# RobotLocomotion/pytorch-dense-correspondence

Hardware: NVIDIA H100
Metric: image-pairs/s (640x480, D=3) fwd+loss+bwd (higher is better)
Workload: dtype f32 (bf16x3 split on the wgmma tensor cores, fp32 accumulate)

## Files before the change

pytorch-dense-correspondence_b200/csrc/conv_tc.cu:

```cuda
#include <cuda.h>
#include <algorithm>
#include <cstring>
#include <functional>
#include <mutex>
#include <unordered_map>

#include "conv.cuh"
#include "conv_tc.cuh"

namespace ddn {

constexpr int TC_BLOCK_K = 64;
constexpr int TC_CONSUMERS = 256;
constexpr int TC_THREADS = TC_CONSUMERS + 32;
constexpr int TC_PRODUCER_WARP = TC_CONSUMERS / 32;
constexpr int TC_WIDE_THREADS = TC_CONSUMERS + 128;
constexpr int TC_A_BYTES = 128 * TC_BLOCK_K * 2;

__device__ __forceinline__ uint32_t smem_u32(const void* p) { return (uint32_t)__cvta_generic_to_shared(p); }

__device__ __forceinline__ void mbar_init(uint32_t bar, uint32_t count) {
  asm volatile("mbarrier.init.shared::cta.b64 [%0], %1;" ::"r"(bar), "r"(count));
}
__device__ __forceinline__ void mbar_expect_tx(uint32_t bar, uint32_t bytes) {
// ... 2 lines not shown
__device__ __forceinline__ void mbar_arrive(uint32_t bar) {
  asm volatile("mbarrier.arrive.shared::cta.b64 _, [%0];" ::"r"(bar) : "memory");
}
__device__ __forceinline__ void mbar_wait(uint32_t bar, uint32_t parity) {
  asm volatile(
      "{\n\t"
      ".reg .pred p;\n\t"
      "WAIT_LOOP:\n\t"
      "mbarrier.try_wait.parity.shared::cta.b64 p, [%0], %1;\n\t"
      "@p bra WAIT_DONE;\n\t"
      "bra WAIT_LOOP;\n\t"
      "WAIT_DONE:\n\t"
      "}\n" ::"r"(bar), "r"(parity) : "memory");
}
__device__ __forceinline__ void fence_barrier_init() { asm volatile("fence.mbarrier_init.release.cluster;" ::: "memory"); }

__device__ __forceinline__ void tma_load_4d(uint32_t dst, const CUtensorMap* map, uint32_t bar, int c0, int c1, int c2, int c3) {
  asm volatile(
      "cp.async.bulk.tensor.4d.shared::cluster.global.mbarrier::complete_tx::bytes [%0], [%1, {%3, %4, %5, %6}], [%2];"
      ::"r"(dst), "l"(map), "r"(bar), "r"(c0), "r"(c1), "r"(c2), "r"(c3) : "memory");
}
__device__ __forceinline__ void tma_load_2d(uint32_t dst, const CUtensorMap* map, uint32_t bar, int c0, int c1) {
  asm volatile(
      "cp.async.bulk.tensor.2d.shared::cluster.global.mbarrier::complete_tx::bytes [%0], [%1, {%3, %4}], [%2];"
      ::"r"(dst), "l"(map), "r"(bar), "r"(c0), "r"(c1) : "memory");
}
__device__ __forceinline__ void tma_prefetch_l2_4d(const CUtensorMap* map, int c0, int c1, int c2, int c3) {
  asm volatile("cp.async.bulk.prefetch.tensor.4d.L2.global.tile [%0, {%1, %2, %3, %4}];" ::"l"(map), "r"(c0), "r"(c1), "r"(c2), "r"(c3) : "memory");
}
__device__ __forceinline__ void tma_prefetch_desc(const CUtensorMap* map) {
  asm volatile("prefetch.tensormap [%0];" ::"l"(map) : "memory");
}

__device__ __forceinline__ uint64_t gmma_desc(uint32_t smem_addr, uint32_t lbo_bytes, uint32_t sbo_bytes) {
  return (uint64_t)((smem_addr >> 4) & 0x3FFF) | ((uint64_t)((lbo_bytes >> 4) & 0x3FFF) << 16) |
         ((uint64_t)((sbo_bytes >> 4) & 0x3FFF) << 32) | ((uint64_t)1 << 62);
}
__device__ __forceinline__ uint64_t gmma_desc_k(uint32_t smem_addr, uint32_t sbo_bytes = 1024) { return gmma_desc(smem_addr, 16, sbo_bytes); }

template <int R>
__device__ __forceinline__ void setmaxnreg_dec() { asm volatile("setmaxnreg.dec.sync.aligned.u32 %0;" ::"n"(R)); }
template <int R>
__device__ __forceinline__ void setmaxnreg_inc() { asm volatile("setmaxnreg.inc.sync.aligned.u32 %0;" ::"n"(R)); }
__device__ __forceinline__ void wgmma_fence() { asm volatile("wgmma.fence.sync.aligned;" ::: "memory"); }
__device__ __forceinline__ void wgmma_commit() { asm volatile("wgmma.commit_group.sync.aligned;" ::: "memory"); }
template <int N>
__device__ __forceinline__ void wgmma_wait() { asm volatile("wgmma.wait_group.sync.aligned %0;" ::"n"(N) : "memory"); }
template <int K>
__device__ __forceinline__ void fence_acc(float (&d)[K]) {
#pragma unroll
  for (int i = 0; i < K; ++i) asm volatile("" : "+f"(d[i])::"memory");
}

template <int N> struct Wgmma;
template <> struct Wgmma<32> {
  template <int TRANS>
  static __device__ __forceinline__ void mma(float (&d)[16], uint64_t a, uint64_t b, int scale_d) {
    asm volatile(
        "{\n.reg .pred p;\nsetp.ne.b32 p, %18, 0;\n"
        "wgmma.mma_async.sync.aligned.m64n32k16.f32.bf16.bf16 {"
        "%0, %1, %2, %3, %4, %5, %6, %7, %8, %9, %10, %11, %12, %13, %14, %15"
        "}, %16, %17, p, 1, 1, %19, %19;\n}\n"
        : "+f"(d[0]), "+f"(d[1]), "+f"(d[2]), "+f"(d[3]), "+f"(d[4]), "+f"(d[5]), "+f"(d[6]), "+f"(d[7]),
          "+f"(d[8]), "+f"(d[9]), "+f"(d[10]), "+f"(d[11]), "+f"(d[12]), "+f"(d[13]), "+f"(d[14]), "+f"(d[15])
        : "l"(a), "l"(b), "r"(scale_d), "n"(TRANS));
  }
};
template <> struct Wgmma<64> {
  template <int TRANS>
// ... 160 lines not shown
        if (!(fmaf(rw[i].x - mu.x, scl.x, be.x) > 0.f)) g.x = 0.f;
        if (!(fmaf(rw[i].y - mu.y, scl.y, be.y) > 0.f)) g.y = 0.f;
        if (!(fmaf(rw[i].z - mu.z, scl.z, be.z) > 0.f)) g.z = 0.f;
        if (!(fmaf(rw[i].w - mu.w, scl.w, be.w) > 0.f)) g.w = 0.f;
      }
      s1.x += g.x; s1.y += g.y; s1.z += g.z; s1.w += g.w;
      s2.x = fmaf(g.x, (rw[i].x - mu.x) * is.x, s2.x); s2.y = fmaf(g.y, (rw[i].y - mu.y) * is.y, s2.y);
      s2.z = fmaf(g.z, (rw[i].z - mu.z) * is.z, s2.z); s2.w = fmaf(g.w, (rw[i].w - mu.w) * is.w, s2.w);
    }
  } else {
#pragma unroll
    for (int i = 0; i < EPI_ROWS; ++i) {
      const float4 raw = i < n_ok ? v[i] : make_float4(0.f, 0.f, 0.f, 0.f);
      if (i < n_ok)
        *reinterpret_cast<float4*>(p.out + off + i * rs) = make_float4(raw.x + adv[i].x, raw.y + adv[i].y, raw.z + adv[i].z, raw.w + adv[i].w);
      s1.x += raw.x; s1.y += raw.y; s1.z += raw.z; s1.w += raw.w;
      s2.x = fmaf(raw.x, raw.x, s2.x); s2.y = fmaf(raw.y, raw.y, s2.y); s2.z = fmaf(raw.z, raw.z, s2.z); s2.w = fmaf(raw.w, raw.w, s2.w);
    }
  }
}

__device__ __forceinline__ void colsum_lane_groups(float4& s1, float4& s2) {
#pragma unroll
  for (int off = 8; off < 32; off <<= 1) {
    s1.x += __shfl_xor_sync(0xffffffffu, s1.x, off); s1.y += __shfl_xor_sync(0xffffffffu, s1.y, off);
    s1.z += __shfl_xor_sync(0xffffffffu, s1.z, off); s1.w += __shfl_xor_sync(0xffffffffu, s1.w, off);
    s2.x += __shfl_xor_sync(0xffffffffu, s2.x, off); s2.y += __shfl_xor_sync(0xffffffffu, s2.y, off);
    s2.z += __shfl_xor_sync(0xffffffffu, s2.z, off); s2.w += __shfl_xor_sync(0xffffffffu, s2.w, off);
  }
}

__device__ __forceinline__ void named_barrier(int id, int threads) { asm volatile("bar.sync %0, %1;" ::"r"(id), "r"(threads) : "memory"); }

__device__ __forceinline__ void conv_epilogue_finalize(const TcEpilogueParams& p, int C, int* s_last, int bar) {
  if (p.fin.a.acc) {
    if (bn_last_cta(p.fin.a.ticket, gridDim.x, threadIdx.x == 0, s_last, [bar] { named_barrier(bar, TC_CONSUMERS); }))
      for (int c = threadIdx.x; c < C; c += TC_CONSUMERS) bn_fwd_finalize_channel(p.fin, c);
  } else if (p.bst.fin.a.acc) {
    if (bn_last_cta(p.bst.fin.a.ticket, gridDim.x, threadIdx.x == 0, s_last, [bar] { named_barrier(bar, TC_CONSUMERS); }))
      for (int c = threadIdx.x; c < C; c += TC_CONSUMERS) bn_bwd_finalize_channel(p.bst.fin, c);
  }
}

struct TcConvParams {
  TcEpilogueParams epi;
  int N, H, W, Cin, Cout;
  int taps_w;
  int dil;
  int stride;
  int tiles_h, tiles_w;
  int n_sub;
  int n_co;
  int full_items, tail_split, total_items;
};

constexpr int TC_SUB_H = 4, TC_SUB_W = 16;
constexpr int TC_SUB_BYTES = 64 * 128;

struct TcItem { int sp, co0, width; };
__device__ __forceinline__ TcItem tc_item(const TcConvParams& p, int idx, int block_n) {
  int tile = idx, piece = 0, width = block_n;
  if (idx >= p.full_items) {
    const int j = idx - p.full_items;
    tile = p.full_items + j / p.tail_split;
    piece = j - (j / p.tail_split) * p.tail_split;
    width = block_n / p.tail_split;
  }
  TcItem it;
  it.sp = tile / p.n_co;
  it.co0 = (tile - it.sp * p.n_co) * block_n + piece * width;
  it.width = width;
  return it;
}
struct TcSub { int n, h0, w0; bool valid; };
__device__ __forceinline__ TcSub tc_sub(const TcConvParams& p, int st) {
  TcSub s;
  s.valid = st < p.n_sub;
  const int tw = st % p.tiles_w; const int t = st / p.tiles_w;
  const int th = t % p.tiles_h;
  s.n = s.valid ? t / p.tiles_h : p.N;
  s.h0 = th * TC_SUB_H; s.w0 = tw * TC_SUB_W;
  return s;
}

template <int W, int BLOCK_N, int NPROD, int STAGES, int TRANS = 0>
__device__ __forceinline__ void conv_tc_mainloop(float (&acc)[W / 2], float (&accx)[W / 2], int num_kb, uint32_t& g, const uint64_t* full_bar,
                                                 const uint64_t* empty_bar, const uint8_t* smem, int wg, int lane) {
  constexpr int NSPLIT = NPROD == 3 ? 2 : 1;
  constexpr int A_BYTES = 128 * TC_BLOCK_K * 2;
  constexpr int B_BYTES = BLOCK_N * TC_BLOCK_K * 2;
  constexpr int STAGE_BYTES = NSPLIT * (A_BYTES + B_BYTES);
  constexpr uint32_t LBO = TRANS ? TC_SUB_BYTES : 16;
  constexpr int K_STEP = TRANS ? 16 * 128 : 32;
  for (int kb = 0; kb < num_kb; ++kb, ++g) {
    const int s = g % STAGES;
    mbar_wait(smem_u32(&full_bar[s]), (g / STAGES) & 1);
    wgmma_fence();
    const uint32_t stg = smem_u32(smem + (size_t)s * STAGE_BYTES);
    const uint64_t a_hi = gmma_desc(stg + wg * TC_SUB_BYTES, LBO, 1024), a_lo = gmma_desc(stg + A_BYTES + wg * TC_SUB_BYTES, LBO, 1024);
    const uint64_t b_hi = gmma_desc(stg + NSPLIT * A_BYTES, LBO, 1024), b_lo = gmma_desc(stg + 2 * A_BYTES + B_BYTES, LBO, 1024);
#pragma unroll
    for (int k = 0; k < TC_BLOCK_K / 16; ++k) {
      const uint64_t adv = (uint64_t)((k * K_STEP) >> 4);
      mma_k16_x<W, TRANS, NPROD>(acc, accx, a_hi + adv, a_lo + adv, b_hi + adv, b_lo + adv, (kb | k) != 0);
    }
    wgmma_commit();
    wgmma_wait<1>();
    if (kb > 0 && lane == 0) mbar_arrive(smem_u32(&empty_bar[(g - 1) % STAGES]));
  }
  wgmma_wait<0>();
  fence_acc(acc);
  if (NPROD == 3) { fence_acc(accx); add_cross(acc, accx); }
  if (lane == 0) mbar_arrive(smem_u32(&empty_bar[(g - 1) % STAGES]));
}

template <int BLOCK_N, int NPROD>
__global__ void __launch_bounds__(TC_WIDE_THREADS, 1)
conv_tc_kernel(const __grid_constant__ CUtensorMap tm_a_hi, const __grid_constant__ CUtensorMap tm_a_lo,
               const __grid_constant__ CUtensorMap tm_b_hi, const __grid_constant__ CUtensorMap tm_b_lo,
               const __grid_constant__ CUtensorMap tm_bt_hi, const __grid_constant__ CUtensorMap tm_bt_lo,
               const TcConvParams p) {
  constexpr int NSPLIT = NPROD == 3 ? 2 : 1;
  constexpr int A_BYTES = 128 * TC_BLOCK_K * 2;
  constexpr int B_BYTES = BLOCK_N * TC_BLOCK_K * 2;
  constexpr int STAGE_BYTES = NSPLIT * (A_BYTES + B_BYTES);
  constexpr int STAGES = (192 * 1024) / STAGE_BYTES >= 8 ? 8 : (192 * 1024) / STAGE_BYTES;
  static_assert(STAGES >= 2, "pipeline needs at least two stages");

  extern __shared__ __align__(1024) uint8_t smem_raw[];
  uint8_t* smem = reinterpret_cast<uint8_t*>((reinterpret_cast<uintptr_t>(smem_raw) + 1023) & ~uintptr_t(1023));
  __shared__ __align__(8) uint64_t full_bar[STAGES];
  __shared__ __align__(8) uint64_t empty_bar[STAGES];
  __shared__ int s_last;
  __shared__ __align__(16) float s_stage[TC_CONSUMERS / 32][EPI_WARP_FLOATS];
  __shared__ __align__(16) float s_part[2][2][4][BLOCK_N];
// ... 68 lines not shown
      const int n_ok = (sb.valid && h < p.H) ? min(EPI_ROWS, p.W - w4) : 0;
      const size_t pix = ((size_t)(n_ok > 0 ? sb.n : 0) * p.H + (n_ok > 0 ? h : 0)) * p.W + (n_ok > 0 ? w4 : 0);
      const size_t cbase = pix * p.Cout + it.co0 + gb * 4;
      const int grp = sb.valid ? sb.n / p.epi.imgs_per_group : 0;
#pragma unroll
      for (int c = 0; c < BLOCK_N / 32; ++c) {
        if (c < (it.width >> 5)) {
          float4 v[EPI_ROWS];
          stage_chunk(acc, c, st, lane, v);
          float4 s1 = make_float4(0.f, 0.f, 0.f, 0.f), s2 = s1;
          conv_epilogue_rows(p.epi, v, cbase + c * 32, (size_t)p.Cout, n_ok, it.co0 + c * 32 + gb * 4, p.Cout, grp, s1, s2);
          if (stats || bstats) {
            colsum_lane_groups(s1, s2);
            if (ga == 0) {
              *reinterpret_cast<float4*>(&s_part[wg][0][w][c * 32 + gb * 4]) = s1;
              *reinterpret_cast<float4*>(&s_part[wg][1][w][c * 32 + gb * 4]) = s2;
            }
          }
        }
      }
      if (stats || bstats) {
        named_barrier(1 + wg, 128);
        if (sb.valid)
          for (int col = e; col < it.width; col += 128) {
#pragma unroll
            for (int k = 0; k < 2; ++k) {
              const float sum = s_part[wg][k][0][col] + s_part[wg][k][1][col] + s_part[wg][k][2][col] + s_part[wg][k][3][col];
              red_add_f64(sum_acc + (size_t)(grp * 2 + k) * p.Cout + it.co0 + col, (double)sum);
            }
          }
        named_barrier(1 + wg, 128);
      }
    }
    conv_epilogue_finalize(p.epi, p.Cout, &s_last, 3);
  }
}

struct TcHaloParams {
  TcEpilogueParams epi;
  int N, H, W;
  int tiles_h, tiles_w, n_tiles;
};
constexpr int HALO_TH = 8, HALO_TW = 16;
constexpr int HALO_BH = HALO_TH + 2, HALO_BW = HALO_TW + 2;
constexpr int HALO_BOX_BYTES = HALO_BH * HALO_BW * 128;
constexpr int HALO_SLOT = ((HALO_BOX_BYTES + 1023) / 1024) * 1024;
constexpr int HALO_B_TAP = 64 * 128;
constexpr int HALO_B_PLANE = 9 * HALO_B_TAP;
__host__ __device__ constexpr int halo_slots(int nprod) { return nprod == 3 ? 2 : 3; }

template <int NPROD>
__global__ void __launch_bounds__(TC_THREADS, 1)
conv64_halo_kernel(const __grid_constant__ CUtensorMap tm_a_hi, const __grid_constant__ CUtensorMap tm_a_lo,
                   const __grid_constant__ CUtensorMap tm_b_hi, const __grid_constant__ CUtensorMap tm_b_lo, const TcHaloParams p) {
  constexpr int NSPLIT = NPROD == 3 ? 2 : 1;
  constexpr int SLOTS = halo_slots(NPROD);
  extern __shared__ __align__(1024) uint8_t smem_raw[];
  uint8_t* smem = reinterpret_cast<uint8_t*>((reinterpret_cast<uintptr_t>(smem_raw) + 1023) & ~uintptr_t(1023));
  uint8_t* smem_b = smem;
  uint8_t* smem_a = smem + NSPLIT * HALO_B_PLANE;
  __shared__ __align__(8) uint64_t full_bar[SLOTS], empty_bar[SLOTS], b_full;
  __shared__ int s_last;
  __shared__ __align__(16) float s_stage[TC_CONSUMERS / 32][EPI_WARP_FLOATS];
  __shared__ __align__(16) float s_part[2][8][64];

  pdl_trigger();
  const int warp = __shfl_sync(0xffffffffu, threadIdx.x >> 5, 0), lane = threadIdx.x & 31;
// ... 108 lines not shown
      fence_acc(acc);
      if (NPROD == 3) { fence_acc(accx); add_cross(acc, accx); }
      if (lane == 0) mbar_arrive(smem_u32(&empty_bar[(g - 1) % SLOTS]));

      const size_t pix0 = ((size_t)n * p.H + h0 + EPI_ROWS * (ga & 1)) * p.W + (w0 + 8 * wg + 2 * w + (ga >> 1));
      const size_t row_stride = (size_t)p.W * 64;
      const int grp = n / p.epi.imgs_per_group;
#pragma unroll
      for (int c = 0; c < 2; ++c) {
        float4 v[EPI_ROWS];
        stage_chunk(acc, c, st, lane, v);
        float4 s1 = make_float4(0.f, 0.f, 0.f, 0.f), s2 = s1;
        conv_epilogue_rows(p.epi, v, pix0 * 64 + gb * 4 + c * 32, row_stride, EPI_ROWS, c * 32 + gb * 4, 64, grp, s1, s2);
        if (stats || bstats) {
          colsum_lane_groups(s1, s2);
          if (ga == 0) {
            *reinterpret_cast<float4*>(&s_part[0][warp][c * 32 + gb * 4]) = s1;
            *reinterpret_cast<float4*>(&s_part[1][warp][c * 32 + gb * 4]) = s2;
          }
        }
      }
      if (stats || bstats) {
        named_barrier(3, TC_CONSUMERS);
        if (threadIdx.x < 128) {
          const int col = threadIdx.x & 63, k = threadIdx.x >> 6;
          float s8 = 0.f;
#pragma unroll
          for (int q = 0; q < 8; ++q) s8 += s_part[k][q][col];
          red_add_f64(sum_acc + (size_t)(grp * 2 + k) * 64 + col, (double)s8);
        }
        named_barrier(3, TC_CONSUMERS);
      }
    }
    conv_epilogue_finalize(p.epi, 64, &s_last, 3);
  }
}

struct TcWgradParams {
  double* dwp;
  int N, H, W, Cin, Cout;
  int taps_w, dil, stride;
  int tiles_h, tiles_w;
  int total_kb;
  int n_co, n_ci, n_tiles;
  int chunks;
};

struct WgradItem { int co0, ci0, tap, kb0, kb1; };
__device__ __forceinline__ WgradItem wgrad_item(const TcWgradParams& p, int idx, int bn) {
  const int c = idx / p.n_tiles;
  int t = idx - c * p.n_tiles;
  WgradItem it;
  it.co0 = (t % p.n_co) * 128; t /= p.n_co;
  it.ci0 = (t % p.n_ci) * bn;
  it.tap = t / p.n_ci;
  it.kb0 = (int)((int64_t)c * p.total_kb / p.chunks);
  it.kb1 = (int)((int64_t)(c + 1) * p.total_kb / p.chunks);
  return it;
}

template <int BN, int NPROD>
__global__ void __launch_bounds__(TC_WIDE_THREADS, 1)
wgrad_tc_kernel(const __grid_constant__ CUtensorMap tm_dy_hi, const __grid_constant__ CUtensorMap tm_dy_lo,
                const __grid_constant__ CUtensorMap tm_x_hi, const __grid_constant__ CUtensorMap tm_x_lo,
                const TcWgradParams p) {
  constexpr int NSPLIT = NPROD == 3 ? 2 : 1;
  constexpr int B_BYTES = BN * TC_BLOCK_K * 2;
// ... 407 lines not shown
                                  const cuuint32_t*, const cuuint32_t*, CUtensorMapInterleave, CUtensorMapSwizzle,
                                  CUtensorMapL2promotion, CUtensorMapFloatOOBfill);

static EncodeTiledFn get_encode_fn() {
  static EncodeTiledFn fn = nullptr;
  static bool tried = false;
  if (!tried) {
    tried = true;
    void* p = nullptr;
    cudaDriverEntryPointQueryResult qres;
    if (cudaGetDriverEntryPoint("cuTensorMapEncodeTiled", &p, cudaEnableDefault, &qres) == cudaSuccess &&
        qres == cudaDriverEntryPointSuccess)
      fn = (EncodeTiledFn)p;
  }
  return fn;
}

struct MapKey {
  const void* base; int d0, d1, d2, d3, b0, b1, b2, sample;
  bool operator==(const MapKey& o) const {
    return base == o.base && d0 == o.d0 && d1 == o.d1 && d2 == o.d2 && d3 == o.d3 && b0 == o.b0 && b1 == o.b1 && b2 == o.b2 && sample == o.sample;
  }
};
struct MapKeyHash {
  size_t operator()(const MapKey& k) const {
    size_t h = std::hash<const void*>()(k.base);
    for (int v : {k.d0, k.d1, k.d2, k.d3, k.b0, k.b1, k.b2, k.sample}) h = h * 1000003u ^ (size_t)v;
    return h;
  }
};
static std::unordered_map<MapKey, CUtensorMap, MapKeyHash> g_maps;
static std::mutex g_maps_mu;

static int make_act_map(CUtensorMap* m, const void* base, int N, int H, int W, int C, int sample = 1) {
  const MapKey key = {base, C, W, H, N, TC_BLOCK_K, TC_SUB_W, TC_SUB_H, sample};
  {
    std::lock_guard<std::mutex> lk(g_maps_mu);
    auto it = g_maps.find(key);
    if (it != g_maps.end()) { *m = it->second; return 0; }
  }
  EncodeTiledFn enc = get_encode_fn();
  if (!enc) { set_error("cuTensorMapEncodeTiled is unavailable (driver too old?)"); return DDN_EUNSUPPORTED; }
  cuuint64_t dims[4] = {(cuuint64_t)C, (cuuint64_t)W, (cuuint64_t)H, (cuuint64_t)N};
  cuuint64_t strides[3] = {(cuuint64_t)C * 2, (cuuint64_t)W * C * 2, (cuuint64_t)H * W * C * 2};
  cuuint32_t box[4] = {(cuuint32_t)TC_BLOCK_K, (cuuint32_t)(TC_SUB_W * sample), (cuuint32_t)(TC_SUB_H * sample), 1};
  cuuint32_t es[4] = {1, (cuuint32_t)sample, (cuuint32_t)sample, 1};
  CUresult r = enc(m, CU_TENSOR_MAP_DATA_TYPE_BFLOAT16, 4, const_cast<void*>(base), dims, strides, box, es,
                   CU_TENSOR_MAP_INTERLEAVE_NONE, CU_TENSOR_MAP_SWIZZLE_128B, CU_TENSOR_MAP_L2_PROMOTION_L2_128B,
                   CU_TENSOR_MAP_FLOAT_OOB_FILL_NONE);
  if (r != CUDA_SUCCESS) { set_error("cuTensorMapEncodeTiled(activations) failed: %d", (int)r); return DDN_EINVAL; }
  std::lock_guard<std::mutex> lk(g_maps_mu);
  if (g_maps.size() > 8192) g_maps.clear();
  g_maps[key] = *m;
  return 0;
}
static int make_act_map_hw(CUtensorMap* m, const void* base, int N, int H, int W, int C, int box_h, int box_w) {
  const MapKey key = {base, C, H, W, N, TC_BLOCK_K, box_h, box_w, -2};
  {
    std::lock_guard<std::mutex> lk(g_maps_mu);
    auto it = g_maps.find(key);
    if (it != g_maps.end()) { *m = it->second; return 0; }
  }
  EncodeTiledFn enc = get_encode_fn();
  if (!enc) { set_error("cuTensorMapEncodeTiled is unavailable (driver too old?)"); return DDN_EUNSUPPORTED; }
  cuuint64_t dims[4] = {(cuuint64_t)C, (cuuint64_t)H, (cuuint64_t)W, (cuuint64_t)N};
  cuuint64_t strides[3] = {(cuuint64_t)W * C * 2, (cuuint64_t)C * 2, (cuuint64_t)H * W * C * 2};
  cuuint32_t box[4] = {(cuuint32_t)TC_BLOCK_K, (cuuint32_t)box_h, (cuuint32_t)box_w, 1};
  cuuint32_t es[4] = {1, 1, 1, 1};
  CUresult r = enc(m, CU_TENSOR_MAP_DATA_TYPE_BFLOAT16, 4, const_cast<void*>(base), dims, strides, box, es,
                   CU_TENSOR_MAP_INTERLEAVE_NONE, CU_TENSOR_MAP_SWIZZLE_128B, CU_TENSOR_MAP_L2_PROMOTION_L2_128B,
                   CU_TENSOR_MAP_FLOAT_OOB_FILL_NONE);
  if (r != CUDA_SUCCESS) { set_error("cuTensorMapEncodeTiled(halo activations) failed: %d", (int)r); return DDN_EINVAL; }
  std::lock_guard<std::mutex> lk(g_maps_mu);
  if (g_maps.size() > 8192) g_maps.clear();
  g_maps[key] = *m;
  return 0;
}
static int make_act_map_halo(CUtensorMap* m, const void* base, int N, int H, int W, int C) {
  return make_act_map_hw(m, base, N, H, W, C, HALO_BH, HALO_BW);
}
static int make_weight_map(CUtensorMap* m, const void* base, int rows, int K, int box_rows) {
  const MapKey key = {base, K, rows, 0, 0, TC_BLOCK_K, box_rows, 0, -1};
  {
    std::lock_guard<std::mutex> lk(g_maps_mu);
    auto it = g_maps.find(key);
    if (it != g_maps.end()) { *m = it->second; return 0; }
  }
  EncodeTiledFn enc = get_encode_fn();
  if (!enc) { set_error("cuTensorMapEncodeTiled is unavailable (driver too old?)"); return DDN_EUNSUPPORTED; }
  cuuint64_t dims[2] = {(cuuint64_t)K, (cuuint64_t)rows};
  cuuint64_t strides[1] = {(cuuint64_t)K * 2};
  cuuint32_t box[2] = {(cuuint32_t)TC_BLOCK_K, (cuuint32_t)box_rows};
  cuuint32_t es[2] = {1, 1};
  CUresult r = enc(m, CU_TENSOR_MAP_DATA_TYPE_BFLOAT16, 2, const_cast<void*>(base), dims, strides, box, es,
                   CU_TENSOR_MAP_INTERLEAVE_NONE, CU_TENSOR_MAP_SWIZZLE_128B, CU_TENSOR_MAP_L2_PROMOTION_L2_256B,
                   CU_TENSOR_MAP_FLOAT_OOB_FILL_NONE);
  if (r != CUDA_SUCCESS) { set_error("cuTensorMapEncodeTiled(weights) failed: %d", (int)r); return DDN_EINVAL; }
  std::lock_guard<std::mutex> lk(g_maps_mu);
  if (g_maps.size() > 8192) g_maps.clear();
  g_maps[key] = *m;
  return 0;
}

template <int BN, int NPROD>
static int launch_wgrad_tc(const CUtensorMap& dy_hi, const CUtensorMap& dy_lo, const CUtensorMap& x_hi, const CUtensorMap& x_lo,
                           const TcWgradParams& p, int workers, cudaStream_t st) {
  constexpr int NSPLIT = NPROD == 3 ? 2 : 1;
  constexpr int STAGE_BYTES = NSPLIT * (TC_A_BYTES + BN * TC_BLOCK_K * 2);
  constexpr int STAGES = (192 * 1024) / STAGE_BYTES >= 8 ? 8 : (192 * 1024) / STAGE_BYTES;
  const size_t smem = (size_t)STAGES * STAGE_BYTES + 1024;
  static bool configured = false;
  if (!configured) {
    DDN_CUDA(cudaFuncSetAttribute(wgrad_tc_kernel<BN, NPROD>, cudaFuncAttributeMaxDynamicSharedMemorySize, (int)smem));
    configured = true;
  }
  DDN_LAUNCH((wgrad_tc_kernel<BN, NPROD>), workers, TC_WIDE_THREADS, smem, st, dy_hi, dy_lo, x_hi, x_lo, p);
  return 0;
}

static int tc_wgrad_chunks(int tiles, int total_kb, int workers) {
  const double even = (double)tiles * total_kb / workers;
  const int max_s = std::max(1, total_kb / 4);
  int best = 1;
  double best_span = 1e300;
  for (int s = 1; s <= max_s; ++s) {
    const double span = (double)ceil_div((int64_t)s * tiles, workers) * (double)ceil_div(total_kb, s);
    if (span <= 1.02 * even) return s;
    if (span < best_span) { best_span = span; best = s; }
// ... 99 lines not shown

int tc_upsample_zero_split(const float* dy, __nv_bfloat16* hi, __nv_bfloat16* lo, int N, int Ho, int Wo, int C, int precision,
                           cudaStream_t st) {
  int64_t total = (int64_t)N * Ho * Wo * (C / 4);
  int blocks = (int)std::min<int64_t>(ceil_div(total, 256), (int64_t)num_sms() * 8);
  DDN_LAUNCH(upsample_zero_split_kernel, blocks, 256, 0, st, dy, hi, lo, N, Ho, Wo, C, precision == DDN_PRECISION_BF16X3 ? 1 : 0);
  return 0;
}

int tc_stem_patches(const float* x_nchw, __nv_bfloat16* hi, __nv_bfloat16* lo, int N, int H, int W, int precision, cudaStream_t st) {
  const int H1 = (H - 1) / 2 + 1, W1 = (W - 1) / 2 + 1;
  DDN_CHECK_ARG(N <= 65535 && H1 <= 65535, "stem: batch / height too large for the launch grid");
  dim3 grid((unsigned)ceil_div(W1, STEM_TW), (unsigned)H1, (unsigned)N);
  DDN_LAUNCH(stem_patch_split_kernel, grid, 256, 0, st, x_nchw, hi, lo, N, H, W, H1, W1, precision == DDN_PRECISION_BF16X3 ? 1 : 0);
  return 0;
}

template <int BLOCK_N, int NPROD>
static int launch_conv_tc(const CUtensorMap& a_hi, const CUtensorMap& a_lo, const CUtensorMap& b_hi, const CUtensorMap& b_lo,
                          const CUtensorMap& bt_hi, const CUtensorMap& bt_lo, const TcConvParams& p, int workers, cudaStream_t st) {
  constexpr int NSPLIT = NPROD == 3 ? 2 : 1;
  constexpr int STAGE_BYTES = NSPLIT * (128 * TC_BLOCK_K * 2 + BLOCK_N * TC_BLOCK_K * 2);
  constexpr int STAGES = (192 * 1024) / STAGE_BYTES >= 8 ? 8 : (192 * 1024) / STAGE_BYTES;
  const size_t smem = (size_t)STAGES * STAGE_BYTES + 1024;
  static bool configured = false;
  if (!configured) {
    DDN_CUDA(cudaFuncSetAttribute(conv_tc_kernel<BLOCK_N, NPROD>, cudaFuncAttributeMaxDynamicSharedMemorySize, (int)smem));
    configured = true;
  }
  DDN_LAUNCH((conv_tc_kernel<BLOCK_N, NPROD>), workers, TC_WIDE_THREADS, smem, st, a_hi, a_lo, b_hi, b_lo, bt_hi, bt_lo, p);
  return 0;
}

template <int NPROD>
static int launch_conv64_halo(const CUtensorMap& a_hi, const CUtensorMap& a_lo, const CUtensorMap& b_hi, const CUtensorMap& b_lo,
                              const TcHaloParams& p, cudaStream_t st) {
  constexpr int NSPLIT = NPROD == 3 ? 2 : 1;
  const size_t smem = (size_t)NSPLIT * HALO_B_PLANE + (size_t)halo_slots(NPROD) * HALO_SLOT + 1024;
  static bool configured = false;
  if (!configured) {
    DDN_CUDA(cudaFuncSetAttribute(conv64_halo_kernel<NPROD>, cudaFuncAttributeMaxDynamicSharedMemorySize, (int)smem));
    configured = true;
  }
  const int grid = std::min(p.n_tiles, tc_worker_sms());
  DDN_LAUNCH((conv64_halo_kernel<NPROD>), grid, TC_THREADS, smem, st, a_hi, a_lo, b_hi, b_lo, p);
  return 0;
}

static int tc_epilogue_request(TcEpilogueParams* e, float* out, const float* addend, const BnFwdFinal* stats, const TcBwdStats* bst,
                               const TcFoldedEpilogue* ep, int N, int gout, int dgrad, int want_lo) {
  memset(e, 0, sizeof(*e));
  e->out = out; e->addend = addend; e->imgs_per_group = N;
  if (stats) {
    DDN_CHECK_ARG(!dgrad && !ep && stats->G >= 1 && stats->G <= BN_MAX_GROUPS && N % stats->G == 0 && stats->C == gout,
                  "bad BatchNorm statistics request");
    e->fin = *stats;
    e->imgs_per_group = N / stats->G;
  }
  if (bst) {
    DDN_CHECK_ARG(dgrad && !ep && !stats && bst->raw && bst->mean && bst->invstd && bst->fin.a.acc && bst->fin.G >= 1 &&
                  bst->fin.G <= BN_MAX_GROUPS && N % bst->fin.G == 0 && bst->fin.C == gout && (bst->y_hi || !bst->relu || (bst->gamma && bst->beta)),
                  "bad BatchNorm backward-statistics request");
    e->bst = *bst;
    e->imgs_per_group = N / bst->fin.G;
  }
  if (ep) {
// ... 32 lines not shown
  if (k == 3 && gin == 64 && gout == 64 && stride == 1 && dil == 1 && Ho % HALO_TH == 0 && Wo % HALO_TW == 0) {
    TcHaloParams hp;
    memset(&hp, 0, sizeof(hp));
    hp.epi = epi; hp.N = N; hp.H = Ho; hp.W = Wo;
    hp.tiles_h = Ho / HALO_TH; hp.tiles_w = Wo / HALO_TW; hp.n_tiles = N * hp.tiles_h * hp.tiles_w;
    CUtensorMap ma_hi, ma_lo, mb_hi, mb_lo;
    DDN_TRY(make_act_map_halo(&ma_hi, in.hi, N, H, W, 64));
    DDN_TRY(make_act_map_halo(&ma_lo, want_lo ? in.lo : in.hi, N, H, W, 64));
    DDN_TRY(make_weight_map(&mb_hi, b_hi, 64, 9 * 64, 64));
    DDN_TRY(make_weight_map(&mb_lo, want_lo ? b_lo : b_hi, 64, 9 * 64, 64));
    ProfScope ps(dgrad ? PROF_CONV_DGRAD_TC : PROF_CONV_FWD_TC, fl, st);
    return want_lo ? launch_conv64_halo<3>(ma_hi, ma_lo, mb_hi, mb_lo, hp, st) : launch_conv64_halo<1>(ma_hi, ma_lo, mb_hi, mb_lo, hp, st);
  }
  const int block_n = gout % 128 == 0 ? 128 : 64;
  TcConvParams p;
  memset(&p, 0, sizeof(p));
  p.epi = epi; p.N = N; p.H = Ho; p.W = Wo; p.Cin = gin; p.Cout = gout; p.taps_w = k; p.dil = dil;
  p.stride = stride;
  p.tiles_h = (int)ceil_div(Ho, TC_SUB_H); p.tiles_w = (int)ceil_div(Wo, TC_SUB_W);
  p.n_sub = N * p.tiles_h * p.tiles_w;
  p.n_co = gout / block_n;
  const int tiles = (int)ceil_div(p.n_sub, 2) * p.n_co;
  const int workers_max = tc_worker_sms();
  const int rem = tiles % workers_max;
  int split = 1;
  if (rem)
    while (split * 2 <= 8 && block_n / (split * 2) >= 32 && rem * split * 2 <= workers_max) split *= 2;
  p.full_items = tiles - rem; p.tail_split = split; p.total_items = p.full_items + rem * split;
  if (split == 1) { p.full_items = tiles; p.total_items = tiles; }
  const int workers = std::min(p.total_items, workers_max);
  const int b_rows = block_n;
  const int bt_rows = b_rows / split;
  CUtensorMap ma_hi, ma_lo, mb_hi, mb_lo, mt_hi, mt_lo;
  DDN_TRY(make_act_map(&ma_hi, in.hi, N, H, W, gin, stride));
  DDN_TRY(make_act_map(&ma_lo, want_lo ? in.lo : in.hi, N, H, W, gin, stride));
  DDN_TRY(make_weight_map(&mb_hi, b_hi, gout, k * k * gin, b_rows));
  DDN_TRY(make_weight_map(&mb_lo, want_lo ? b_lo : b_hi, gout, k * k * gin, b_rows));
  DDN_TRY(make_weight_map(&mt_hi, b_hi, gout, k * k * gin, bt_rows));
  DDN_TRY(make_weight_map(&mt_lo, want_lo ? b_lo : b_hi, gout, k * k * gin, bt_rows));
  ProfScope ps(dgrad ? PROF_CONV_DGRAD_TC : PROF_CONV_FWD_TC, fl, st);
#define CONV_TC(BN)                                                                                                           \
  (want_lo ? launch_conv_tc<BN, 3>(ma_hi, ma_lo, mb_hi, mb_lo, mt_hi, mt_lo, p, workers, st)                                   \
           : launch_conv_tc<BN, 1>(ma_hi, ma_lo, mb_hi, mb_lo, mt_hi, mt_lo, p, workers, st))
  if (block_n == 128) return CONV_TC(128);
  return CONV_TC(64);
#undef CONV_TC
}

int tc_dgrad_strided(const float* dy_f32, TcPlanes up, const float* w_oihw, const TcPlanes* w_packed, float* dx, const float* addend,
                     int N, int H, int W, int Cin, int Cout, int k, int precision, void* wws, size_t wws_bytes, cudaStream_t st,
                     const TcBwdStats* bst) {
  DDN_TRY(tc_upsample_zero_split(dy_f32, const_cast<__nv_bfloat16*>(up.hi), const_cast<__nv_bfloat16*>(up.lo), N, H / 2, W / 2, Cout,
                                 precision, st));
  return tc_conv_planes(up, w_oihw, w_packed, dx, addend, nullptr, N, H, W, Cin, Cout, k, 1, 1, 1, precision, wws, wws_bytes, st, nullptr, bst);
}

int tc_stem_pack_weights(const float* w_conv1, __nv_bfloat16* hi, __nv_bfloat16* lo, int precision, cudaStream_t st) {
  DDN_LAUNCH(stem_pack_weights_kernel, (64 * 192 + 255) / 256, 256, 0, st, w_conv1, hi, lo, precision == DDN_PRECISION_BF16X3 ? 1 : 0);
  return 0;
}
int tc_stem_forward(TcPlanes patches, const float* w_conv1, const TcPlanes* w_packed, float* raw, const BnFwdFinal* stats, int N, int H1,
                    int W1, int precision, void* wws, size_t wws_bytes, cudaStream_t st) {
  TcPlanes wpk;
  if (w_packed) wpk = *w_packed;
  else {
    char* base = reinterpret_cast<char*>(align_up(reinterpret_cast<uintptr_t>(wws), 1024));
    DDN_CHECK_ARG((size_t)(base - (char*)wws) + 2 * 64 * 192 * 2 + 1024 <= wws_bytes, "weight staging too small");
    __nv_bfloat16* ph = (__nv_bfloat16*)base; __nv_bfloat16* pl = (__nv_bfloat16*)(base + align_up((size_t)64 * 192 * 2, 1024));
    DDN_TRY(tc_stem_pack_weights(w_conv1, ph, pl, precision, st));
    wpk.hi = ph; wpk.lo = pl;
  }
  return tc_conv_planes(patches, nullptr, &wpk, raw, nullptr, stats, N, H1, W1, 192, 64, 1, 1, 1, 0, precision, wws, wws_bytes, st);
}

int tc_stem_wgrad(TcPlanes patches, TcPlanes dy, int N, int H1, int W1, int precision, double* dwp, cudaStream_t st) {
  return tc_wgrad_planes(patches, dy, nullptr, N, H1, W1, 192, 64, 1, 1, 1, precision, dwp, st);
}

// ... 61 lines not shown
```

Before: 140.6.

## Add dgrad conv kernel with dedicated epilogue warpgroup via smem handoff

Adds a warp-specialized dgrad convolution kernel in which two consumer warpgroups run the wgmma mainloop and a separate epilogue warpgroup drains accumulators from a shared-memory handoff buffer. This lets the epilogue (stores, BN stats reduction) overlap the next tile's MMA work. To fit the handoff buffer and a deep ring, the k-block shrinks to 32 channels with 64B swizzle TMA maps and matching wgmma descriptors. The costs are a lower MMA-per-barrier ratio, extra shared-memory traffic for the handoff, and tighter register budgets.

```diff
diff --git a/pytorch-dense-correspondence_b200/csrc/conv_tc.cu b/pytorch-dense-correspondence_b200/csrc/conv_tc.cu
--- a/pytorch-dense-correspondence_b200/csrc/conv_tc.cu
+++ b/pytorch-dense-correspondence_b200/csrc/conv_tc.cu
@@ -58,9 +58,9 @@
   asm volatile("prefetch.tensormap [%0];" ::"l"(map) : "memory");
 }
 
-__device__ __forceinline__ uint64_t gmma_desc(uint32_t smem_addr, uint32_t lbo_bytes, uint32_t sbo_bytes) {
+__device__ __forceinline__ uint64_t gmma_desc(uint32_t smem_addr, uint32_t lbo_bytes, uint32_t sbo_bytes, uint32_t layout = 1) {
   return (uint64_t)((smem_addr >> 4) & 0x3FFF) | ((uint64_t)((lbo_bytes >> 4) & 0x3FFF) << 16) |
-         ((uint64_t)((sbo_bytes >> 4) & 0x3FFF) << 32) | ((uint64_t)1 << 62);
+         ((uint64_t)((sbo_bytes >> 4) & 0x3FFF) << 32) | ((uint64_t)layout << 62);
 }
 __device__ __forceinline__ uint64_t gmma_desc_k(uint32_t smem_addr, uint32_t sbo_bytes = 1024) { return gmma_desc(smem_addr, 16, sbo_bytes); }
 
@@ -287,13 +287,13 @@
 
 __device__ __forceinline__ void named_barrier(int id, int threads) { asm volatile("bar.sync %0, %1;" ::"r"(id), "r"(threads) : "memory"); }
 
-__device__ __forceinline__ void conv_epilogue_finalize(const TcEpilogueParams& p, int C, int* s_last, int bar) {
+__device__ __forceinline__ void conv_epilogue_finalize(const TcEpilogueParams& p, int C, int* s_last, int bar, int tid, int nthreads) {
   if (p.fin.a.acc) {
-    if (bn_last_cta(p.fin.a.ticket, gridDim.x, threadIdx.x == 0, s_last, [bar] { named_barrier(bar, TC_CONSUMERS); }))
-      for (int c = threadIdx.x; c < C; c += TC_CONSUMERS) bn_fwd_finalize_channel(p.fin, c);
+    if (bn_last_cta(p.fin.a.ticket, gridDim.x, tid == 0, s_last, [bar, nthreads] { named_barrier(bar, nthreads); }))
+      for (int c = tid; c < C; c += nthreads) bn_fwd_finalize_channel(p.fin, c);
   } else if (p.bst.fin.a.acc) {
-    if (bn_last_cta(p.bst.fin.a.ticket, gridDim.x, threadIdx.x == 0, s_last, [bar] { named_barrier(bar, TC_CONSUMERS); }))
-      for (int c = threadIdx.x; c < C; c += TC_CONSUMERS) bn_bwd_finalize_channel(p.bst.fin, c);
+    if (bn_last_cta(p.bst.fin.a.ticket, gridDim.x, tid == 0, s_last, [bar, nthreads] { named_barrier(bar, nthreads); }))
+      for (int c = tid; c < C; c += nthreads) bn_bwd_finalize_channel(p.bst.fin, c);
   }
 }
 
@@ -338,24 +338,27 @@
   return s;
 }
 
-template <int W, int BLOCK_N, int NPROD, int STAGES, int TRANS = 0>
+template <int W, int BLOCK_N, int NPROD, int STAGES, int TRANS = 0, int BLOCK_K = TC_BLOCK_K>
 __device__ __forceinline__ void conv_tc_mainloop(float (&acc)[W / 2], float (&accx)[W / 2], int num_kb, uint32_t& g, const uint64_t* full_bar,
                                                  const uint64_t* empty_bar, const uint8_t* smem, int wg, int lane) {
+  static_assert(BLOCK_K == 64 || (BLOCK_K == 32 && !TRANS), "k-block: 64 channels, or 32 with K-major operands");
   constexpr int NSPLIT = NPROD == 3 ? 2 : 1;
-  constexpr int A_BYTES = 128 * TC_BLOCK_K * 2;
-  constexpr int B_BYTES = BLOCK_N * TC_BLOCK_K * 2;
+  constexpr int A_BYTES = 128 * BLOCK_K * 2;
+  constexpr int B_BYTES = BLOCK_N * BLOCK_K * 2;
   constexpr int STAGE_BYTES = NSPLIT * (A_BYTES + B_BYTES);
-  constexpr uint32_t LBO = TRANS ? TC_SUB_BYTES : 16;
+  constexpr uint32_t SUB_BYTES = 64 * BLOCK_K * 2;
+  constexpr uint32_t LBO = TRANS ? SUB_BYTES : 16;
+  constexpr uint32_t SBO = 8 * BLOCK_K * 2, LAYOUT = BLOCK_K == 64 ? 1 : 2;
   constexpr int K_STEP = TRANS ? 16 * 128 : 32;
   for (int kb = 0; kb < num_kb; ++kb, ++g) {
     const int s = g % STAGES;
     mbar_wait(smem_u32(&full_bar[s]), (g / STAGES) & 1);
     wgmma_fence();
     const uint32_t stg = smem_u32(smem + (size_t)s * STAGE_BYTES);
-    const uint64_t a_hi = gmma_desc(stg + wg * TC_SUB_BYTES, LBO, 1024), a_lo = gmma_desc(stg + A_BYTES + wg * TC_SUB_BYTES, LBO, 1024);
-    const uint64_t b_hi = gmma_desc(stg + NSPLIT * A_BYTES, LBO, 1024), b_lo = gmma_desc(stg + 2 * A_BYTES + B_BYTES, LBO, 1024);
-#pragma unroll
-    for (int k = 0; k < TC_BLOCK_K / 16; ++k) {
+    const uint64_t a_hi = gmma_desc(stg + wg * SUB_BYTES, LBO, SBO, LAYOUT), a_lo = gmma_desc(stg + A_BYTES + wg * SUB_BYTES, LBO, SBO, LAYOUT);
+    const uint64_t b_hi = gmma_desc(stg + NSPLIT * A_BYTES, LBO, SBO, LAYOUT), b_lo = gmma_desc(stg + 2 * A_BYTES + B_BYTES, LBO, SBO, LAYOUT);
+#pragma unroll
+    for (int k = 0; k < BLOCK_K / 16; ++k) {
       const uint64_t adv = (uint64_t)((k * K_STEP) >> 4);
       mma_k16_x<W, TRANS, NPROD>(acc, accx, a_hi + adv, a_lo + adv, b_hi + adv, b_lo + adv, (kb | k) != 0);
     }
@@ -490,7 +493,193 @@
         named_barrier(1 + wg, 128);
       }
     }
-    conv_epilogue_finalize(p.epi, p.Cout, &s_last, 3);
+    conv_epilogue_finalize(p.epi, p.Cout, &s_last, 3, threadIdx.x, TC_CONSUMERS);
+  }
+}
+
+constexpr int TC_HANDOFF_BLOCK_K = 32;
+constexpr int TC_HANDOFF_THREADS = TC_CONSUMERS + 256;
+constexpr int TC_EPI_WARP0 = TC_CONSUMERS / 32;
+constexpr int TC_HANDOFF_PRODUCER_WARP = TC_EPI_WARP0 + 4;
+constexpr int TC_REG_CONSUMER = 168, TC_REG_EPILOGUE = 136, TC_REG_PRODUCER = 40;
+static_assert(TC_CONSUMERS * TC_REG_CONSUMER + 128 * (TC_REG_EPILOGUE + TC_REG_PRODUCER) <= 65536, "register file overcommitted");
+constexpr int TC_SMEM_LIMIT = 227 * 1024;
+
+template <int BLOCK_N, int NPROD>
+struct TcHandoffSmem {
+  static constexpr int NSPLIT = NPROD == 3 ? 2 : 1;
+  static constexpr int A_BYTES = 128 * TC_HANDOFF_BLOCK_K * 2;
+  static constexpr int SUB_BYTES = 64 * TC_HANDOFF_BLOCK_K * 2;
+  static constexpr int B_BYTES = BLOCK_N * TC_HANDOFF_BLOCK_K * 2;
+  static constexpr int STAGE_BYTES = NSPLIT * (A_BYTES + B_BYTES);
+  static constexpr int HANDOFF_STRIDE = BLOCK_N + 8;
+  static constexpr int HANDOFF_WARP = 16 * HANDOFF_STRIDE;
+  static constexpr int HANDOFF_BYTES = TC_CONSUMERS / 32 * HANDOFF_WARP * 4;
+  static constexpr int STATIC_BYTES = 2 * 2 * 4 * BLOCK_N * 4 + 1024;
+  static constexpr int RING_MAX = (TC_SMEM_LIMIT - STATIC_BYTES - HANDOFF_BYTES - 1024) / STAGE_BYTES;
+  static constexpr int STAGES = RING_MAX >= 8 ? 8 : RING_MAX;
+  static constexpr int DYNAMIC_BYTES = STAGES * STAGE_BYTES + HANDOFF_BYTES + 1024;
+  static_assert(STAGES >= 4, "the ring needs at least four stages");
+  static_assert(DYNAMIC_BYTES + STATIC_BYTES <= TC_SMEM_LIMIT, "shared memory over the per-block limit");
+};
+
+template <int W, int K>
+__device__ __forceinline__ void handoff_write(const float (&acc)[K], float* st, int stride, int lane) {
+  const int r = lane >> 2, q = (lane & 3) * 2;
+#pragma unroll
+  for (int j = 0; j < W / 8; ++j) {
+    *reinterpret_cast<float2*>(st + r * stride + 8 * j + q) = make_float2(acc[4 * j], acc[4 * j + 1]);
+    *reinterpret_cast<float2*>(st + (r + 8) * stride + 8 * j + q) = make_float2(acc[4 * j + 2], acc[4 * j + 3]);
+  }
+}
+
+template <int BLOCK_N, int NPROD>
+__global__ void __launch_bounds__(TC_HANDOFF_THREADS, 1)
+conv_tc_handoff_kernel(const __grid_constant__ CUtensorMap tm_a_hi, const __grid_constant__ CUtensorMap tm_a_lo,
+               const __grid_constant__ CUtensorMap tm_b_hi, const __grid_constant__ CUtensorMap tm_b_lo,
+               const __grid_constant__ CUtensorMap tm_bt_hi, const __grid_constant__ CUtensorMap tm_bt_lo,
+               const TcConvParams p) {
+  using SM = TcHandoffSmem<BLOCK_N, NPROD>;
+  constexpr int NSPLIT = SM::NSPLIT, A_BYTES = SM::A_BYTES, B_BYTES = SM::B_BYTES, SUB_BYTES = SM::SUB_BYTES;
+  constexpr int STAGE_BYTES = SM::STAGE_BYTES, STAGES = SM::STAGES;
+
+  extern __shared__ __align__(1024) uint8_t smem_raw[];
+  uint8_t* smem = reinterpret_cast<uint8_t*>((reinterpret_cast<uintptr_t>(smem_raw) + 1023) & ~uintptr_t(1023));
+  float* const handoff = reinterpret_cast<float*>(smem + STAGES * STAGE_BYTES);
+  __shared__ __align__(8) uint64_t full_bar[STAGES];
+  __shared__ __align__(8) uint64_t empty_bar[STAGES];
+  __shared__ __align__(8) uint64_t handoff_full, handoff_empty;
+  __shared__ int s_last;
+  __shared__ __align__(16) float s_part[2][2][4][BLOCK_N];
+
+  pdl_trigger();
+  const int warp = __shfl_sync(0xffffffffu, threadIdx.x >> 5, 0), lane = threadIdx.x & 31;
+  const int cin_chunks = p.Cin / TC_HANDOFF_BLOCK_K;
+  const int num_kb = p.taps_w * p.taps_w * cin_chunks;
+  const int half = p.taps_w >> 1;
+
+  if (threadIdx.x == 0) {
+    for (int s = 0; s < STAGES; ++s) { mbar_init(smem_u32(&full_bar[s]), 1); mbar_init(smem_u32(&empty_bar[s]), TC_CONSUMERS / 32); }
+    mbar_init(smem_u32(&handoff_full), TC_CONSUMERS);
+    mbar_init(smem_u32(&handoff_empty), 128);
+    fence_barrier_init();
+    tma_prefetch_desc(&tm_a_hi); tma_prefetch_desc(&tm_b_hi); tma_prefetch_desc(&tm_bt_hi);
+    if (NSPLIT == 2) { tma_prefetch_desc(&tm_a_lo); tma_prefetch_desc(&tm_b_lo); tma_prefetch_desc(&tm_bt_lo); }
+  }
+  __syncthreads();
+  pdl_wait();
+
+  if (warp >= TC_HANDOFF_PRODUCER_WARP) {
+    setmaxnreg_dec<TC_REG_PRODUCER>();
+    if (warp == TC_HANDOFF_PRODUCER_WARP && lane == 0) {
+      uint32_t g = 0;
+      for (int idx = blockIdx.x; idx < p.total_items; idx += gridDim.x) {
+        const TcItem it = tc_item(p, idx, BLOCK_N);
+        const bool tail = it.width != BLOCK_N;
+        const uint32_t stage_tx = (uint32_t)(NSPLIT * (A_BYTES + it.width * TC_HANDOFF_BLOCK_K * 2));
+        const CUtensorMap* mb_hi = tail ? &tm_bt_hi : &tm_b_hi;
+        const CUtensorMap* mb_lo = tail ? &tm_bt_lo : &tm_b_lo;
+        const TcSub s0 = tc_sub(p, it.sp * 2), s1 = tc_sub(p, it.sp * 2 + 1);
+        for (int kb = 0; kb < num_kb; ++kb, ++g) {
+          const int s = g % STAGES;
+          mbar_wait(smem_u32(&empty_bar[s]), ((g / STAGES) & 1) ^ 1);
+          const int tap = kb / cin_chunks, cc = kb - tap * cin_chunks;
+          const int r = tap / p.taps_w, sx = tap - r * p.taps_w;
+          const int dh = (r - half) * p.dil, dw = (sx - half) * p.dil;
+          uint8_t* stg = smem + (size_t)s * STAGE_BYTES;
+          const uint32_t bar = smem_u32(&full_bar[s]);
+          mbar_expect_tx(bar, stage_tx);
+          tma_load_4d(smem_u32(stg), &tm_a_hi, bar, cc * TC_HANDOFF_BLOCK_K, s0.w0 * p.stride + dw, s0.h0 * p.stride + dh, s0.n);
+          tma_load_4d(smem_u32(stg + SUB_BYTES), &tm_a_hi, bar, cc * TC_HANDOFF_BLOCK_K, s1.w0 * p.stride + dw, s1.h0 * p.stride + dh, s1.n);
+          tma_load_2d(smem_u32(stg + NSPLIT * A_BYTES), mb_hi, bar, kb * TC_HANDOFF_BLOCK_K, it.co0);
+          if (NSPLIT == 2) {
+            tma_load_4d(smem_u32(stg + A_BYTES), &tm_a_lo, bar, cc * TC_HANDOFF_BLOCK_K, s0.w0 * p.stride + dw, s0.h0 * p.stride + dh, s0.n);
+            tma_load_4d(smem_u32(stg + A_BYTES + SUB_BYTES), &tm_a_lo, bar, cc * TC_HANDOFF_BLOCK_K, s1.w0 * p.stride + dw, s1.h0 * p.stride + dh, s1.n);
+            tma_load_2d(smem_u32(stg + 2 * A_BYTES + B_BYTES), mb_lo, bar, kb * TC_HANDOFF_BLOCK_K, it.co0);
+          }
+        }
+      }
+    }
+  } else if (warp >= TC_EPI_WARP0) {
+    setmaxnreg_inc<TC_REG_EPILOGUE>();
+    const int w = warp - TC_EPI_WARP0, e = threadIdx.x - TC_CONSUMERS;
+    const int ga = lane >> 3, gb = lane & 7;
+    const bool stats = p.epi.fin.a.acc != nullptr;
+    const bool bstats = p.epi.bst.fin.a.acc != nullptr;
+    double* const sum_acc = bstats ? p.epi.bst.fin.a.acc : p.epi.fin.a.acc;
+    uint32_t n = 0;
+    for (int idx = blockIdx.x; idx < p.total_items; idx += gridDim.x, ++n) {
+      const TcItem it = tc_item(p, idx, BLOCK_N);
+      mbar_wait(smem_u32(&handoff_full), n & 1);
+#pragma unroll 1
+      for (int wg = 0; wg < 2; ++wg) {
+        const TcSub sb = tc_sub(p, it.sp * 2 + wg);
+        const int h = sb.h0 + w, w4 = sb.w0 + EPI_ROWS * ga;
+        const int n_ok = (sb.valid && h < p.H) ? min(EPI_ROWS, p.W - w4) : 0;
+        const size_t pix = ((size_t)(n_ok > 0 ? sb.n : 0) * p.H + (n_ok > 0 ? h : 0)) * p.W + (n_ok > 0 ? w4 : 0);
+        const size_t cbase = pix * p.Cout + it.co0 + gb * 4;
+        const int grp = sb.valid ? sb.n / p.epi.imgs_per_group : 0;
+        const float* st = handoff + (4 * wg + w) * SM::HANDOFF_WARP + EPI_ROWS * ga * SM::HANDOFF_STRIDE + 4 * gb;
+#pragma unroll
+        for (int c = 0; c < BLOCK_N / 32; ++c) {
+          if (c < (it.width >> 5)) {
+            float4 v[EPI_ROWS];
+#pragma unroll
+            for (int i = 0; i < EPI_ROWS; ++i) v[i] = *reinterpret_cast<const float4*>(st + i * SM::HANDOFF_STRIDE + 32 * c);
+            float4 s1 = make_float4(0.f, 0.f, 0.f, 0.f), s2 = s1;
+            conv_epilogue_rows(p.epi, v, cbase + c * 32, (size_t)p.Cout, n_ok, it.co0 + c * 32 + gb * 4, p.Cout, grp, s1, s2);
+            if (stats || bstats) {
+              colsum_lane_groups(s1, s2);
+              if (ga == 0) {
+                *reinterpret_cast<float4*>(&s_part[wg][0][w][c * 32 + gb * 4]) = s1;
+                *reinterpret_cast<float4*>(&s_part[wg][1][w][c * 32 + gb * 4]) = s2;
+              }
+            }
+          }
+        }
+      }
+      mbar_arrive(smem_u32(&handoff_empty));
+      if (stats || bstats) {
+        named_barrier(1, 128);
+        for (int wg = 0; wg < 2; ++wg) {
+          const TcSub sb = tc_sub(p, it.sp * 2 + wg);
+          const int grp = sb.valid ? sb.n / p.epi.imgs_per_group : 0;
+          if (sb.valid)
+            for (int col = e; col < it.width; col += 128) {
+#pragma unroll
+              for (int k = 0; k < 2; ++k) {
+                const float sum = s_part[wg][k][0][col] + s_part[wg][k][1][col] + s_part[wg][k][2][col] + s_part[wg][k][3][col];
+                red_add_f64(sum_acc + (size_t)(grp * 2 + k) * p.Cout + it.co0 + col, (double)sum);
+              }
+            }
+        }
+        named_barrier(1, 128);
+      }
+    }
+    conv_epilogue_finalize(p.epi, p.Cout, &s_last, 2, e, 128);
+  } else {
+    setmaxnreg_inc<TC_REG_CONSUMER>();
+    const int wg = warp >> 2;
+    float* const ho = handoff + warp * SM::HANDOFF_WARP;
+    float acc[BLOCK_N / 2], accx[BLOCK_N / 2];
+    uint32_t g = 0, n = 0;
+    for (int idx = blockIdx.x; idx < p.total_items; idx += gridDim.x, ++n) {
+      const TcItem it = tc_item(p, idx, BLOCK_N);
+      if (it.width == BLOCK_N) {
+        conv_tc_mainloop<BLOCK_N, BLOCK_N, NPROD, STAGES, 0, TC_HANDOFF_BLOCK_K>(acc, accx, num_kb, g, full_bar, empty_bar, smem, wg, lane);
+        mbar_wait(smem_u32(&handoff_empty), (n & 1) ^ 1);
+        handoff_write<BLOCK_N>(acc, ho, SM::HANDOFF_STRIDE, lane);
+      } else if (BLOCK_N > 64 && it.width == 64) {
+        conv_tc_mainloop<64, BLOCK_N, NPROD, STAGES, 0, TC_HANDOFF_BLOCK_K>(acc_cols<64>(acc), acc_cols<64>(accx), num_kb, g, full_bar, empty_bar, smem, wg, lane);
+        mbar_wait(smem_u32(&handoff_empty), (n & 1) ^ 1);
+        handoff_write<64>(acc, ho, SM::HANDOFF_STRIDE, lane);
+      } else {
+        conv_tc_mainloop<32, BLOCK_N, NPROD, STAGES, 0, TC_HANDOFF_BLOCK_K>(acc_cols<32>(acc), acc_cols<32>(accx), num_kb, g, full_bar, empty_bar, smem, wg, lane);
+        mbar_wait(smem_u32(&handoff_empty), (n & 1) ^ 1);
+        handoff_write<32>(acc, ho, SM::HANDOFF_STRIDE, lane);
+      }
+      mbar_arrive(smem_u32(&handoff_full));
+    }
   }
 }
 
@@ -665,7 +854,7 @@
         named_barrier(3, TC_CONSUMERS);
       }
     }
-    conv_epilogue_finalize(p.epi, 64, &s_last, 3);
+    conv_epilogue_finalize(p.epi, 64, &s_last, 3, threadIdx.x, TC_CONSUMERS);
   }
 }
 
@@ -1139,8 +1328,8 @@
 static std::unordered_map<MapKey, CUtensorMap, MapKeyHash> g_maps;
 static std::mutex g_maps_mu;
 
-static int make_act_map(CUtensorMap* m, const void* base, int N, int H, int W, int C, int sample = 1) {
-  const MapKey key = {base, C, W, H, N, TC_BLOCK_K, TC_SUB_W, TC_SUB_H, sample};
+static int make_act_map(CUtensorMap* m, const void* base, int N, int H, int W, int C, int sample = 1, int box_k = TC_BLOCK_K) {
+  const MapKey key = {base, C, W, H, N, box_k, TC_SUB_W, TC_SUB_H, sample};
   {
     std::lock_guard<std::mutex> lk(g_maps_mu);
     auto it = g_maps.find(key);
@@ -1150,10 +1339,10 @@
   if (!enc) { set_error("cuTensorMapEncodeTiled is unavailable (driver too old?)"); return DDN_EUNSUPPORTED; }
   cuuint64_t dims[4] = {(cuuint64_t)C, (cuuint64_t)W, (cuuint64_t)H, (cuuint64_t)N};
   cuuint64_t strides[3] = {(cuuint64_t)C * 2, (cuuint64_t)W * C * 2, (cuuint64_t)H * W * C * 2};
-  cuuint32_t box[4] = {(cuuint32_t)TC_BLOCK_K, (cuuint32_t)(TC_SUB_W * sample), (cuuint32_t)(TC_SUB_H * sample), 1};
+  cuuint32_t box[4] = {(cuuint32_t)box_k, (cuuint32_t)(TC_SUB_W * sample), (cuuint32_t)(TC_SUB_H * sample), 1};
   cuuint32_t es[4] = {1, (cuuint32_t)sample, (cuuint32_t)sample, 1};
   CUresult r = enc(m, CU_TENSOR_MAP_DATA_TYPE_BFLOAT16, 4, const_cast<void*>(base), dims, strides, box, es,
-                   CU_TENSOR_MAP_INTERLEAVE_NONE, CU_TENSOR_MAP_SWIZZLE_128B, CU_TENSOR_MAP_L2_PROMOTION_L2_128B,
+                   CU_TENSOR_MAP_INTERLEAVE_NONE, box_k == 64 ? CU_TENSOR_MAP_SWIZZLE_128B : CU_TENSOR_MAP_SWIZZLE_64B, CU_TENSOR_MAP_L2_PROMOTION_L2_128B,
                    CU_TENSOR_MAP_FLOAT_OOB_FILL_NONE);
   if (r != CUDA_SUCCESS) { set_error("cuTensorMapEncodeTiled(activations) failed: %d", (int)r); return DDN_EINVAL; }
   std::lock_guard<std::mutex> lk(g_maps_mu);
@@ -1186,8 +1375,8 @@
 static int make_act_map_halo(CUtensorMap* m, const void* base, int N, int H, int W, int C) {
   return make_act_map_hw(m, base, N, H, W, C, HALO_BH, HALO_BW);
 }
-static int make_weight_map(CUtensorMap* m, const void* base, int rows, int K, int box_rows) {
-  const MapKey key = {base, K, rows, 0, 0, TC_BLOCK_K, box_rows, 0, -1};
+static int make_weight_map(CUtensorMap* m, const void* base, int rows, int K, int box_rows, int box_k = TC_BLOCK_K) {
+  const MapKey key = {base, K, rows, 0, 0, box_k, box_rows, 0, -1};
   {
     std::lock_guard<std::mutex> lk(g_maps_mu);
     auto it = g_maps.find(key);
@@ -1197,10 +1386,10 @@
   if (!enc) { set_error("cuTensorMapEncodeTiled is unavailable (driver too old?)"); return DDN_EUNSUPPORTED; }
   cuuint64_t dims[2] = {(cuuint64_t)K, (cuuint64_t)rows};
   cuuint64_t strides[1] = {(cuuint64_t)K * 2};
-  cuuint32_t box[2] = {(cuuint32_t)TC_BLOCK_K, (cuuint32_t)box_rows};
+  cuuint32_t box[2] = {(cuuint32_t)box_k, (cuuint32_t)box_rows};
   cuuint32_t es[2] = {1, 1};
   CUresult r = enc(m, CU_TENSOR_MAP_DATA_TYPE_BFLOAT16, 2, const_cast<void*>(base), dims, strides, box, es,
-                   CU_TENSOR_MAP_INTERLEAVE_NONE, CU_TENSOR_MAP_SWIZZLE_128B, CU_TENSOR_MAP_L2_PROMOTION_L2_256B,
+                   CU_TENSOR_MAP_INTERLEAVE_NONE, box_k == 64 ? CU_TENSOR_MAP_SWIZZLE_128B : CU_TENSOR_MAP_SWIZZLE_64B, CU_TENSOR_MAP_L2_PROMOTION_L2_256B,
                    CU_TENSOR_MAP_FLOAT_OOB_FILL_NONE);
   if (r != CUDA_SUCCESS) { set_error("cuTensorMapEncodeTiled(weights) failed: %d", (int)r); return DDN_EINVAL; }
   std::lock_guard<std::mutex> lk(g_maps_mu);
@@ -1366,6 +1555,28 @@
   return 0;
 }
 
+template <int BLOCK_N, int NPROD>
+static int launch_conv_tc_handoff(const CUtensorMap& a_hi, const CUtensorMap& a_lo, const CUtensorMap& b_hi, const CUtensorMap& b_lo,
+                          const CUtensorMap& bt_hi, const CUtensorMap& bt_lo, const TcConvParams& p, int workers, cudaStream_t st) {
+  const size_t smem = TcHandoffSmem<BLOCK_N, NPROD>::DYNAMIC_BYTES;
+  static bool configured = false;
+  if (!configured) {
+    cudaFuncAttributes fa;
+    DDN_CUDA(cudaFuncGetAttributes(&fa, conv_tc_handoff_kernel<BLOCK_N, NPROD>));
+    int dev = 0, optin = 0;
+    DDN_CUDA(cudaGetDevice(&dev));
+    DDN_CUDA(cudaDeviceGetAttribute(&optin, cudaDevAttrMaxSharedMemoryPerBlockOptin, dev));
+    if (smem + fa.sharedSizeBytes > (size_t)optin) {
+      set_error("conv_tc_handoff_kernel needs %zu bytes of shared memory, the device allows %d", smem + fa.sharedSizeBytes, optin);
+      return DDN_EUNSUPPORTED;
+    }
+    DDN_CUDA(cudaFuncSetAttribute(conv_tc_handoff_kernel<BLOCK_N, NPROD>, cudaFuncAttributeMaxDynamicSharedMemorySize, (int)smem));
+    configured = true;
+  }
+  DDN_LAUNCH((conv_tc_handoff_kernel<BLOCK_N, NPROD>), workers, TC_HANDOFF_THREADS, smem, st, a_hi, a_lo, b_hi, b_lo, bt_hi, bt_lo, p);
+  return 0;
+}
+
 template <int NPROD>
 static int launch_conv64_halo(const CUtensorMap& a_hi, const CUtensorMap& a_lo, const CUtensorMap& b_hi, const CUtensorMap& b_lo,
                               const TcHaloParams& p, cudaStream_t st) {
@@ -1464,18 +1675,19 @@
   const int b_rows = block_n;
   const int bt_rows = b_rows / split;
   CUtensorMap ma_hi, ma_lo, mb_hi, mb_lo, mt_hi, mt_lo;
-  DDN_TRY(make_act_map(&ma_hi, in.hi, N, H, W, gin, stride));
-  DDN_TRY(make_act_map(&ma_lo, want_lo ? in.lo : in.hi, N, H, W, gin, stride));
-  DDN_TRY(make_weight_map(&mb_hi, b_hi, gout, k * k * gin, b_rows));
-  DDN_TRY(make_weight_map(&mb_lo, want_lo ? b_lo : b_hi, gout, k * k * gin, b_rows));
-  DDN_TRY(make_weight_map(&mt_hi, b_hi, gout, k * k * gin, bt_rows));
-  DDN_TRY(make_weight_map(&mt_lo, want_lo ? b_lo : b_hi, gout, k * k * gin, bt_rows));
+  const int box_k = dgrad ? TC_HANDOFF_BLOCK_K : TC_BLOCK_K;
+  DDN_TRY(make_act_map(&ma_hi, in.hi, N, H, W, gin, stride, box_k));
+  DDN_TRY(make_act_map(&ma_lo, want_lo ? in.lo : in.hi, N, H, W, gin, stride, box_k));
+  DDN_TRY(make_weight_map(&mb_hi, b_hi, gout, k * k * gin, b_rows, box_k));
+  DDN_TRY(make_weight_map(&mb_lo, want_lo ? b_lo : b_hi, gout, k * k * gin, b_rows, box_k));
+  DDN_TRY(make_weight_map(&mt_hi, b_hi, gout, k * k * gin, bt_rows, box_k));
+  DDN_TRY(make_weight_map(&mt_lo, want_lo ? b_lo : b_hi, gout, k * k * gin, bt_rows, box_k));
   ProfScope ps(dgrad ? PROF_CONV_DGRAD_TC : PROF_CONV_FWD_TC, fl, st);
-#define CONV_TC(BN)                                                                                                           \
-  (want_lo ? launch_conv_tc<BN, 3>(ma_hi, ma_lo, mb_hi, mb_lo, mt_hi, mt_lo, p, workers, st)                                   \
-           : launch_conv_tc<BN, 1>(ma_hi, ma_lo, mb_hi, mb_lo, mt_hi, mt_lo, p, workers, st))
-  if (block_n == 128) return CONV_TC(128);
-  return CONV_TC(64);
+#define CONV_TC(L, BN)                                                                                                        \
+  (want_lo ? L<BN, 3>(ma_hi, ma_lo, mb_hi, mb_lo, mt_hi, mt_lo, p, workers, st)                                                \
+           : L<BN, 1>(ma_hi, ma_lo, mb_hi, mb_lo, mt_hi, mt_lo, p, workers, st))
+  if (dgrad) return block_n == 128 ? CONV_TC(launch_conv_tc_handoff, 128) : CONV_TC(launch_conv_tc_handoff, 64);
+  return block_n == 128 ? CONV_TC(launch_conv_tc, 128) : CONV_TC(launch_conv_tc, 64);
 #undef CONV_TC
 }
 
```

Result: no change. 141.4, median of 6 (+0.6%).
